# innnky/vispeech

Measured on AMD Instinct MI355X. Metric: 44.1kHz samples/sec, higher is better.
Workload: dtype f32 (split-f16 MFMA, 3-term); 1 GPU; C3: 64 mixed zh/ja utterances (~5 s each) per GPU, 44.1 kHz, hop 512, phoneme/duration/F0/energy/noise supplied, random-init (synthetic) weights of configs/config.json; 2 batches in flight per GPU; utterances_per_gpu=64, global_batch=64, padded_frames=489, frames_padded=31296, frames_computed=28902, parallelism=shard1, generator=f16s, controls=all, batches_in_flight=2

## Files before the change

### vispeech_amd/csrc/api_common.h

```cpp
#pragma once
#include <algorithm>
#include <cmath>
#include <cstdlib>
#include <cstring>
#include <vector>

#include "model.h"
#include "row_controls.h"

namespace vsp {

struct T3 {
  float* p = nullptr;
  long bs = 0, cs = 0;
  T3 chan(int c) const { return T3{p ? p + (size_t)c * cs : nullptr, bs, cs}; }
};

struct Ws {
  char* base;
  size_t cap;
  size_t cur = 0;
  bool dry;
  bool overflow = false;
  Ws(void* b, size_t c, bool d) : base((char*)b), cap(c), dry(d) {}
// ... 35 lines not shown
  const int* glen = nullptr;
  int grate_in = 0, grate_out = 0;
  bool iso = false;
  double work_frac = 1.0;
  bool dry() const { return ws.dry; }
  const float* A(size_t off) const { return ctx->arena + off; }
  bool ok() const { return rc == VSP_OK && !ws.overflow; }
  void chk(hipError_t e, const char* what) {
    if (e != hipSuccess && rc == VSP_OK) rc = ctx->fail(VSP_ERR_HIP, "%s: %s", what, hipGetErrorString(e));
  }

  static int fam(int kind, int channels) {
    if (channels <= 16) return kind | (7 << 3);
    int l = 0;
    while ((32 << l) < channels && l < 7) ++l;
    return kind | (l << 3);
  }
  ConvArgs args(const Conv& L, T3 x, T3 out, int T_in, int Nq) const {
    ConvArgs a;
    std::memset(&a, 0, sizeof a);
    a.x = x.p; a.x_bs = x.bs; a.x_cs = x.cs;
    a.wp = A(L.w);
    a.bias = L.b >= 0 ? A((size_t)L.b) : nullptr;
    a.out = out.p; a.o_bs = out.bs; a.o_cs = out.cs;
    a.Cin = L.Cin; a.M = L.M; a.K = L.K; a.dil = L.dil; a.pad = L.pad;
    a.T_in = T_in; a.Nq = Nq;
    a.nchunks = (L.Cin + CONV_CK - 1) / CONV_CK;
    a.alpha = 1.f; a.div = 1.f;
    a.ups_s = L.ups_s; a.ups_p = L.ups_p;
    a.f16s = L.f16s ? 1 : 0;
    a.wg = (L.has_wg && ctx->cols) ? reinterpret_cast<const uint16_t*>(A(L.wg)) : nullptr;
    a.wg_max_blocks = ctx->cols_blocks;
    a.wg_min_blocks = ctx->cols_min_blocks;
    return a;
  }
  bool prof_begin(int cls, int fam = VSP_FAM_OTHER) {
    if (!ctx->prof_on) return false;
    while (ctx->ev_pool.size() < ctx->ev_used + 2) {
      hipEvent_t e;
      if (hipEventCreate(&e) != hipSuccess) { rc = ctx->fail(VSP_ERR_HIP, "hipEventCreate"); return false; }
      ctx->ev_pool.push_back(e);
    }
    if (ctx->ev_cls.size() < ctx->ev_pool.size() / 2) {
      ctx->ev_cls.resize(ctx->ev_pool.size() / 2, 0);
      ctx->ev_fam.resize(ctx->ev_pool.size() / 2, 0);
      ctx->ev_flops.resize(ctx->ev_pool.size() / 2, 0.0);
      ctx->ev_bytes.resize(ctx->ev_pool.size() / 2, 0.0);
      ctx->ev_moved.resize(ctx->ev_pool.size() / 2, 0.0);
    }
    ctx->ev_cls[ctx->ev_used / 2] = cls;
    ctx->ev_fam[ctx->ev_used / 2] = fam;
    (void)hipEventRecord(ctx->ev_pool[ctx->ev_used], s);
    return true;
  }
  void prof_end(int cls, double flops, double bytes, double bytes_ext, double bytes_moved) {
    (void)hipEventRecord(ctx->ev_pool[ctx->ev_used + 1], s);
    const double f = cls == VSP_PROF_GENERATOR ? work_frac : 1.0;
    ctx->ev_flops[ctx->ev_used / 2] = flops * f;
    ctx->ev_bytes[ctx->ev_used / 2] = bytes * f;
    ctx->ev_moved[ctx->ev_used / 2] = bytes_moved * f;
    ctx->ev_used += 2;
    ctx->prof_launches[cls] += 1;
    ctx->prof_flops[cls] += flops * f;
    ctx->prof_bytes[cls] += bytes * f;
    ctx->prof_bytes_ext[cls] += bytes_ext * f;
    ctx->prof_bytes_moved[cls] += bytes_moved * f;
// ... 121 lines not shown
```

### vispeech_amd/csrc/api_context.hip

```cpp
#include "api_common.h"

using namespace vsp;

namespace vsp {

int check_ready(vsp_ctx* ctx) {
  if (!ctx) return VSP_ERR_ARG;
  if (!ctx->ready) return ctx->fail(VSP_ERR_STATE, "weights not finalised");
  return VSP_OK;
}

int check_vc(vsp_ctx* ctx) {
  const int rc = check_ready(ctx);
  if (rc) return rc;
  if (ctx->cfg.spec_channels <= 0) return ctx->fail(VSP_ERR_STATE, "context was created without spec_channels");
  if (!ctx->model.has_vc) return ctx->fail(VSP_ERR_STATE, "enc_q.* tensors were not loaded before vsp_finalize_weights");
  return VSP_OK;
}

}

extern "C" {

int vsp_abi_version(void) { return VSP_ABI_VERSION; }

int vsp_create(const vsp_config* cfg, int device, vsp_ctx** out) { return vsp_create_ex(cfg, 1, device, out); }

int vsp_create_ex(const vsp_config* cfg, int32_t resblock, int device, vsp_ctx** out) {
  if (!cfg || !out || (resblock != 1 && resblock != 2)) return VSP_ERR_ARG;
  vsp_ctx* ctx = new (std::nothrow) vsp_ctx();
  if (!ctx) return VSP_ERR_ARG;
  ctx->cfg = *cfg;
  ctx->resblock = resblock;
  ctx->device = device;
  if (const char* e = getenv("VSP_FRAME")) ctx->frame_f16s = strcmp(e, "f32") != 0;
  if (const char* e = getenv("VSP_ATT")) ctx->att_f16s = strcmp(e, "f32") != 0;
  bool want_f16 = false;
  if (const char* e = getenv("VSP_GENERATOR")) {
    if (!strcmp(e, "f32")) ctx->gen_mode = 0;
    want_f16 = !strcmp(e, "f16");
  }
  if (const char* e = getenv("VSP_FUSE_PAIRS")) ctx->fuse_pairs = atoi(e) != 0;
  if (const char* e = getenv("VSP_RB2_FUSE")) ctx->rb2_fuse = atoi(e) != 0;
  if (const char* e = getenv("VSP_TIMG")) ctx->t_img = atoi(e) != 0;
  if (const char* e = getenv("VSP_PP")) ctx->pp_pairs = atoi(e) != 0;
  if (const char* e = getenv("VSP_PAIR")) ctx->pair_ring = !strcmp(e, "ring");
  if (const char* e = getenv("VSP_CHAIN_RING")) ctx->chain_ring = atoi(e) != 0;
  if (const char* e = getenv("VSP_CHAIN")) ctx->chain_mask = atoi(e);
  if (const char* e = getenv("VSP_RW64")) ctx->rw64 = atoi(e) != 0;
  if (const char* e = getenv("VSP_TRIM_TAILS")) ctx->trim_tails = atoi(e) != 0;
  if (const char* e = getenv("VSP_TAIL_TABLE")) ctx->tail_table_on = atoi(e) != 0;
  if (const char* e = getenv("VSP_COLS")) ctx->cols = atoi(e) != 0;
  if (const char* e = getenv("VSP_COLS_BLOCKS")) ctx->cols_blocks = atol(e);
  if (const char* e = getenv("VSP_COLS_MIN_BLOCKS")) ctx->cols_min_blocks = atol(e);
  if (const char* e = getenv("VSP_ACT_SCALE_LOG2")) {
    const int l = atoi(e);
    ctx->act_scale = std::ldexp(1.f, l < 0 ? 0 : l > 8 ? 8 : l);
  }
  if (const char* e = getenv("VSP_EARLY_FL")) ctx->early_fl = atoi(e) != 0;
  if (const char* e = getenv("VSP_RB_STREAMS")) ctx->rb_streams = atoi(e);
#ifdef VSP_EXPERIMENTS
  if (const char* e = getenv("VSP_ATT_KSPLIT")) ctx->att_ksplit = atoi(e);
  if (const char* e = getenv("VSP_CHUNK_MB")) ctx->chunk_mb = atof(e);
  if (const char* e = getenv("VSP_CHAIN_CH")) ctx->chain_ch = atoi(e);
  if (const char* e = getenv("VSP_CHAIN128")) ctx->chain128_mask = atoi(e);
#endif
  build_schema(ctx->cfg, ctx->schema, ctx->resblock);
  const int rc = plan_model(ctx);
  if (want_f16 && ctx->gen_mode == 1) ctx->gen_mode = 2;
  *out = ctx;
  return rc;
}

int vsp_destroy(vsp_ctx* ctx) {
  if (!ctx) return VSP_ERR_ARG;
  for (auto e : ctx->ev_pool) (void)hipEventDestroy(e);
  for (auto e : ctx->sync_ev) (void)hipEventDestroy(e);
  if (ctx->fl_ev) (void)hipEventDestroy(ctx->fl_ev);
  if (ctx->fl_pinned) (void)hipHostFree(ctx->fl_pinned);
  if (ctx->flags_host) (void)hipHostFree(ctx->flags_host);
  for (auto st : ctx->side) if (st) (void)hipStreamDestroy(st);
  if (ctx->arena && ctx->arena_owned) (void)hipFree(ctx->arena);
  if (ctx->out_stage.tab) (void)hipFree(ctx->out_stage.tab);
  tail_table_drop(ctx);
  for (auto& r : ctx->in_rates) if (r.tab) (void)hipFree(r.tab);
// ... 436 lines not shown
```

### vispeech_amd/csrc/conv_mfma.hip

```cpp
#include "kernels.h"

#include <cstdio>
#include <cstdlib>
#include <cstring>
#include <type_traits>

namespace vsp {

typedef float f32x16 __attribute__((ext_vector_type(16)));

size_t packed_conv_floats(int M, int Cin, int K) {
  const size_t mt = (M + 31) / 32, nc = (Cin + CONV_CK - 1) / CONV_CK;
  return mt * nc * (size_t)K * 1024;
}

void pack_conv_weights(float* dst, int M, int Cin, int K, const float* dense) {
  const int nc = (Cin + CONV_CK - 1) / CONV_CK;
  std::memset(dst, 0, packed_conv_floats(M, Cin, K) * sizeof(float));
  for (int row = 0; row < M; ++row) {
    const int mtile = row >> 5, rin = row & 31;
    for (int ci = 0; ci < Cin; ++ci) {
      const int chunk = ci / CONV_CK, cc = ci % CONV_CK;
      const int kk = cc >> 1, hh = cc & 1, lane = rin + 32 * hh, kg = kk >> 2, i = kk & 3;
      for (int tap = 0; tap < K; ++tap) {
        const size_t idx =
            (((((size_t)mtile * nc + chunk) * K + tap) * (CONV_CK / 8) + kg) * 64 + lane) * 4 + i;
        dst[idx] = dense[((size_t)row * Cin + ci) * K + tap];
      }
    }
  }
}

void pack_conv_weights_f16s(float* dst_f, int M, int Cin, int K, const float* dense) {
// ... 420 lines not shown
    for (int nt = 0; nt < NT; ++nt) {
      const int tq = t0 + (wn * NT + nt) * 32;
      if constexpr (S == 1) {
        const int mtile = mtile0 + ms;
        if (mtile < n_mtiles && conv_tile_lean_ok(a, mtile)) {
          conv_tile_lean(a, acc[ms][nt], mtile, tq, l31, h, b, len);
          continue;
        }
      } else if constexpr (S == 2) {
        const int mtile = mtile0 + 2 * ms;
        if (conv_gate_lean_ok(a, mtile, n_mtiles)) {
          conv_gate_lean(a, acc[2 * ms][nt], acc[2 * ms + 1][nt], mtile, tq, l31, h, b, len);
          continue;
        }
      }
      f32x16 t[S][1];
#pragma unroll
      for (int u = 0; u < S; ++u) t[u][0] = acc[S * ms + u][nt];
      ConvEpi<S, 1> e;
      conv_epi_load<S, 1, false>(a, e, mtile0 + S * ms, n_mtiles, tq, 0, l31, h, b);
      conv_epi_store<S, 1>(a, t, e, mtile0 + S * ms, n_mtiles, tq, 0, l31, h, b, len);
    }
}
template <int MT, int NT>
__device__ __forceinline__ void conv_store_plain(const ConvArgs& a, f32x16 (&acc)[MT][NT], int mtile0, int n_mtiles, int t0,
                                                 int wn, int l31, int h, int b, int len) {
  if (a.act == 2) {
    if constexpr (MT % 2 == 0) conv_store_slices<2, MT, NT>(a, acc, mtile0, n_mtiles, t0, wn, l31, h, b, len);
  } else {
    conv_store_slices<1, MT, NT>(a, acc, mtile0, n_mtiles, t0, wn, l31, h, b, len);
  }
}

template <int MT, int NT, int WM, int WN, bool F16S, bool RING = false, bool PRUNE = false>
__global__ void __launch_bounds__(64 * WM * WN, F16S ? 2 : 1) conv1d_f32_mfma(ConvArgs a) {
  static_assert(!RING || F16S, "the weight ring serves the split-f16 path");
  static_assert(!PRUNE || (F16S && RING), "the pruned form is the split-f16 ring kernel");
  constexpr int BN = 32 * NT * WN;
  constexpr int LWP = BN + CONV_HALO;
  constexpr int NW = WM * WN;
  constexpr int KG = CONV_CK / 8;
  extern __shared__ __attribute__((aligned(16))) float xs[];
  constexpr int SB = MT * WM * 4096;
  constexpr int NS = conv_ring_slots(MT, WM), DEPTH = NS - 1;
  constexpr int PW = MT * WM * 4 / NW;
  static_assert(!RING || (MT * WM * 4) % NW == 0, "pieces divide over the waves");
  [[maybe_unused]] char* const ring = reinterpret_cast<char*>(xs) + (size_t)CONV_CK * LWP * sizeof(float);

  const int tid = threadIdx.x;
  const int wave = __builtin_amdgcn_readfirstlane(tid >> 6);
  const int lane = tid & 63;
  const int l31 = lane & 31, h = lane >> 5;
  const int wm = wave / WN, wn = wave % WN;
  const int b = blockIdx.z;
  const int t0 = blockIdx.x * BN;
  const int mtile0 = (blockIdx.y * WM + wm) * MT;
  const int n_mtiles = (a.M + 31) >> 5;
  const int len = a.lengths ? (int)a.lengths[b] : 0x7fffffff;
  const int LW = BN + (a.K - 1) * a.dil;
  const int total_it = a.nchunks * a.K;

  f32x16 acc[MT][NT];
#pragma unroll
  for (int mt = 0; mt < MT; ++mt)
#pragma unroll
    for (int nt = 0; nt < NT; ++nt)
#pragma unroll
      for (int r = 0; r < 16; ++r) {
        acc[mt][nt][r] = 0.f;
      }
// ... 368 lines not shown
        const int row = mtile * 32 + (r & 3) + 8 * (r >> 2) + 4 * h;
        if (!st[r]) continue;
        float v = acc[mt][nt][r];
        if (a.bias) v += a.bias[row];
        if (condb) v += condb[row];
        if (a.act == 1) v = fmaxf(v, 0.f);
        if (a.mask_pre && !valid) v = 0.f;
        if (a.alpha != 1.f) v *= a.alpha;
        if (resb) v += rv[r];
        if (a.acc_prev) v += pv[r];
        conv_div(v, a.div);
        if (a.mask_post && !valid) v = 0.f;
        outb[oidx[r]] = v;
      }
    }
  }
}

constexpr int FR_HALO = 12;

#define FR_VM1(k) case k: asm volatile("s_waitcnt vmcnt(" #k ")" ::: "memory"); break;
#define FR_VM8(a, b, c, d, e, f, g, h) FR_VM1(a) FR_VM1(b) FR_VM1(c) FR_VM1(d) FR_VM1(e) FR_VM1(f) FR_VM1(g) FR_VM1(h)
#ifndef FR_DIAG
#define FR_DIAG 0
#endif
__device__ __forceinline__ void fr_vmcnt(int n) {
  if constexpr ((FR_DIAG & 2) != 0) return;
  switch (n) {
    FR_VM8(0, 1, 2, 3, 4, 5, 6, 7) FR_VM8(8, 9, 10, 11, 12, 13, 14, 15) FR_VM8(16, 17, 18, 19, 20, 21, 22, 23)
    FR_VM8(24, 25, 26, 27, 28, 29, 30, 31) FR_VM8(32, 33, 34, 35, 36, 37, 38, 39) FR_VM8(40, 41, 42, 43, 44, 45, 46, 47)
    FR_VM8(48, 49, 50, 51, 52, 53, 54, 55) FR_VM8(56, 57, 58, 59, 60, 61, 62, 63)
    default: asm volatile("s_waitcnt vmcnt(63)" ::: "memory"); break;
  }
}
#ifdef FR_STAMPS
constexpr int FR_NSTAMP = 512, FR_NSAMPLE = 64;
__device__ unsigned long long g_fr_stamps[FR_NSAMPLE][FR_NSTAMP];
__device__ unsigned g_fr_stamp_count;
__device__ int g_fr_stamp_on;
#define FR_STAMPT(tag)                                                                  \
  do {                                                                                  \
    if (stamp_slot >= 0 && stamp_n < FR_NSTAMP && lane == 0)                            \
      g_fr_stamps[stamp_slot][stamp_n] = (__builtin_amdgcn_s_memrealtime() & 0x00ffffffffffffffull) | ((unsigned long long)(tag) << 56); \
    ++stamp_n;                                                                          \
  } while (0)
extern "C" int vsp_debug_stamps_frame(unsigned long long* host, int max_samples, int reset) {
  unsigned n = 0;
  (void)hipDeviceSynchronize();
  (void)hipMemcpyFromSymbol(&n, HIP_SYMBOL(g_fr_stamp_count), sizeof n);
  if ((int)n > max_samples) n = max_samples;
  if (n > (unsigned)FR_NSAMPLE) n = FR_NSAMPLE;
  (void)hipMemcpyFromSymbol(host, HIP_SYMBOL(g_fr_stamps), (size_t)n * FR_NSTAMP * sizeof(unsigned long long));
  if (reset) { const unsigned z = 0; (void)hipMemcpyToSymbol(HIP_SYMBOL(g_fr_stamp_count), &z, sizeof z); }
  return (int)n;
}
#else
#define FR_STAMPT(tag) ((void)0)
#endif
#if FR_DIAG & 1
#define FR_MFMA16(a, b, c) ([&]() { asm volatile("" ::"v"(a), "v"(b)); return c; }())
#else
#define FR_MFMA16(a, b, c) __builtin_amdgcn_mfma_f32_32x32x16_f16(a, b, c, 0, 0, 0)
#endif

template <int MT, int NT, int WM, int WN, int K, int G, int RI, int WI>
__global__ void __launch_bounds__(64 * WM * WN, 1) conv_frame_f16s(ConvArgs a) {
// ... 273 lines not shown
template <int MT, int NT, int WM, int WN, int K, int G, int RI, int WI>
static hipError_t launch_frame(const ConvArgs& a, int B, hipStream_t s) {
  constexpr int BN = 32 * NT * WN, BM = 32 * MT * WM, NW = WM * WN;
  constexpr int NF4 = CONV_CK * ((BN + (K == 1 ? 0 : FR_HALO)) / 4);
  constexpr size_t lds = (size_t)WI * G * ((NF4 + 64 * NW - 1) / (64 * NW)) * NW * 1024 + (size_t)RI * G * K * MT * WM * 4096;
  static_assert(lds <= 160 * 1024, "LDS budget");
  static std::atomic<uint64_t> attr_done{0};
  auto kern = conv_frame_f16s<MT, NT, WM, WN, K, G, RI, WI>;
  if (hipError_t e = set_max_dynamic_lds(reinterpret_cast<const void*>(kern), (int)lds, attr_done); e != hipSuccess) return e;
  dim3 grid((a.Nq + BN - 1) / BN, (a.M + BM - 1) / BM, B);
#ifdef FR_STAMPS
  {
    static int target = -2;
    if (target == -2) { const char* e = getenv("VSP_STAMP_FRAME"); target = e ? atoi(e) : -1; }
    const int on = g_fr_launch_no++ == target ? 1 : 0;
    (void)hipMemcpyToSymbolAsync(HIP_SYMBOL(g_fr_stamp_on), &g_fr_on_vals[on], sizeof(int), 0, hipMemcpyHostToDevice, s);
    if (on) fprintf(stderr, "[stamps] conv_frame_f16s<%d,%d,%d,%d,K%d,G%d,%d,%d> M %d Cin %d Nq %d grid %u x %u x %u\n", MT, NT, WM, WN, K,
                    G, RI, WI, a.M, a.Cin, a.Nq, grid.x, grid.y, grid.z);
  }
#endif
  hipLaunchKernelGGL(kern, grid, dim3(64 * WM * WN), lds, s, a);
  return hipGetLastError();
}
template <int MT, int NT, int WM, int WN>
static bool launch_frame_k(const ConvArgs& a, int B, hipStream_t s, hipError_t& e) {
  switch (a.K) {
    case 1: e = launch_frame<MT, NT, WM, WN, 1, 2, 3, 3>(a, B, s); return true;
    case 3: e = launch_frame<MT, NT, WM, WN, 3, 1, 3, 3>(a, B, s); return true;
    case 5: e = launch_frame<MT, NT, WM, WN, 5, 1, 2, 3>(a, B, s); return true;
    default: return false;
  }
}

template <int MT, int NT, int WM, int WN, bool F16S = false, bool RING = false, bool PRUNE = false>
static hipError_t launch_tile(const ConvArgs& a, int B, hipStream_t s) {
  constexpr int BN = 32 * NT * WN, BM = 32 * MT * WM;
  constexpr size_t lds = (size_t)CONV_CK * (BN + CONV_HALO) * sizeof(float) +
                         (RING ? (size_t)conv_ring_slots(MT, WM) * MT * WM * 4096 : 0);
  static_assert(lds <= 160 * 1024, "LDS budget (<= 80 KiB: two blocks per CU)");
  static std::atomic<uint64_t> attr_done{0};
  auto kern = conv1d_f32_mfma<MT, NT, WM, WN, F16S, RING, PRUNE>;
  if (hipError_t e = set_max_dynamic_lds(reinterpret_cast<const void*>(kern), (int)lds, attr_done); e != hipSuccess) return e;
  dim3 grid((a.Nq + BN - 1) / BN, (a.M + BM - 1) / BM, B);
  hipLaunchKernelGGL(kern, grid, dim3(64 * WM * WN), lds, s, a);
  return hipGetLastError();
}

template <int K, bool GATE>
__global__ void __launch_bounds__(256, 1) conv_frame_splitk(ConvArgs a) {
  constexpr int MT = 2, NT = 1, NWV = 4;
  constexpr int HALO = K == 1 ? 0 : FR_HALO;
  constexpr int BN = 32 * NT, LWP = BN + HALO, LWP4 = LWP / 4;
  constexpr int WBUF = CONV_CK * LWP * 4;
  constexpr int NIT = (16 * LWP4 + 63) / 64;
  constexpr int GT = 2;
  constexpr int GPC = (K + GT - 1) / GT;
  extern __shared__ __attribute__((aligned(16))) float xs[];
  char* const wbase = reinterpret_cast<char*>(xs);

  const int tid = threadIdx.x;
  const int wave = __builtin_amdgcn_readfirstlane(tid >> 6);
  const int lane = tid & 63;
  const int l31 = lane & 31, h = lane >> 5;
  const int b = blockIdx.z;
  const int t0 = blockIdx.x * BN;
  const int mtile0 = blockIdx.y * MT;
  const int n_mtiles = (a.M + 31) >> 5;
  const int nch = a.nchunks;
  const int total_it = nch * K;
  constexpr int FM = GATE ? 2 : 1;
  ConvEpi<FM, 1> epi;
  const bool finisher = wave < (GATE ? 1 : 2);
  const int fmt0 = mtile0 + (GATE ? 0 : wave);
  if (finisher) conv_epi_load<FM, 1>(a, epi, fmt0, n_mtiles, t0, 0, l31, h, b, 1);

// ... 315 lines not shown
      return form_tile(2, 1, 1, 4, true, true);
    }
    if (prune_ok) return form_tile(2, 2, 2, 2, true, true, true);
    return form_tile(2, 2, 2, 2, true, true);
  }
  if (a.f16s) {
    if (a.ups_s > 0) return form_of(VSP_CONV_FORM_NONE);
    if (a.M <= 32 && !gate) {
      if (a.Nq >= 1024) return form_tile(1, 4, 1, 4, true);
      return form_tile(1, 1, 1, 2, true);
    }
    if (a.Nq <= 96) return form_tile(2, 1, 1, 2, true);
    if (a.M <= 64 || (a.M % 128 != 0 && a.M < 256)) {
      if (a.Nq >= 1024) return form_tile(2, 2, 1, 4, true);
      return form_tile(2, 1, 1, 4, true);
    }
    return form_tile(2, 2, 2, 2, true);
  }
  if (a.M <= 32 && !gate) {
    if (a.Nq >= 1024) return form_tile(1, 4, 1, 4);
    return form_tile(1, 1, 1, 2);
  }
  if (a.Nq <= 96) return form_tile(2, 1, 1, 2);
  if (a.M <= 64 || (a.M % 128 != 0 && a.M < 256)) {
    if (a.Nq >= 1024) return form_tile(2, 4, 1, 4);
    return form_tile(2, 1, 1, 4);
  }
  return form_tile(2, 2, 2, 2);
}

static hipError_t launch_tile_form(const ConvForm& f, const ConvArgs& a, int B, hipStream_t s) {
  const int shape = f.mt * 1000 + f.nt * 100 + f.wm * 10 + f.wn;
  if (f.prune) {
    switch (shape) {
      case 2114: return launch_tile<2, 1, 1, 4, true, true, true>(a, B, s);
      case 2222: return launch_tile<2, 2, 2, 2, true, true, true>(a, B, s);
    }
  } else if (f.ring) {
    switch (shape) {
      case 1414: return launch_tile<1, 4, 1, 4, true, true>(a, B, s);
      case 1112: return launch_tile<1, 1, 1, 2, true, true>(a, B, s);
      case 2112: return launch_tile<2, 1, 1, 2, true, true>(a, B, s);
      case 2214: return launch_tile<2, 2, 1, 4, true, true>(a, B, s);
      case 2114: return launch_tile<2, 1, 1, 4, true, true>(a, B, s);
      case 2222: return launch_tile<2, 2, 2, 2, true, true>(a, B, s);
    }
  } else if (f.f16s) {
    switch (shape) {
      case 1414: return launch_tile<1, 4, 1, 4, true>(a, B, s);
      case 1112: return launch_tile<1, 1, 1, 2, true>(a, B, s);
      case 2112: return launch_tile<2, 1, 1, 2, true>(a, B, s);
      case 2214: return launch_tile<2, 2, 1, 4, true>(a, B, s);
      case 2114: return launch_tile<2, 1, 1, 4, true>(a, B, s);
      case 2222: return launch_tile<2, 2, 2, 2, true>(a, B, s);
    }
  } else {
    switch (shape) {
      case 1414: return launch_tile<1, 4, 1, 4>(a, B, s);
      case 1112: return launch_tile<1, 1, 1, 2>(a, B, s);
      case 2112: return launch_tile<2, 1, 1, 2>(a, B, s);
      case 2414: return launch_tile<2, 4, 1, 4>(a, B, s);
      case 2114: return launch_tile<2, 1, 1, 4>(a, B, s);
      case 2222: return launch_tile<2, 2, 2, 2>(a, B, s);
    }
  }
  return hipErrorInvalidValue;
// ... 26 lines not shown
```

### vispeech_amd/csrc/kernels.h

```cpp
#pragma once
#include <hip/hip_runtime.h>
#include <stdint.h>

#include <atomic>

#include "../../include/vispeech_hip.h"

namespace vsp {

inline hipError_t set_max_dynamic_lds(const void* kern, int bytes, std::atomic<uint64_t>& done) {
  int dev = 0;
  hipError_t e = hipGetDevice(&dev);
  if (e != hipSuccess) return e;
  const uint64_t bit = 1ull << (dev & 63);
  if (done.load(std::memory_order_acquire) & bit) return hipSuccess;
  e = hipFuncSetAttribute(kern, hipFuncAttributeMaxDynamicSharedMemorySize, bytes);
  if (e == hipSuccess) done.fetch_or(bit, std::memory_order_release);
  return e;
}

constexpr int CONV_CK = 32;
constexpr int CONV_HALO = 64;

struct ConvArgs {
  const float* x; long x_bs, x_cs;
  const float* wp;
  const float* bias;
  float* out; long o_bs, o_cs;
  const float* res; long r_bs, r_cs;
  const float* cond; long cond_bs;
  const int64_t* lengths;
  int Cin, M, K, dil, pad;
  int T_in;
  int Nq;
  int nchunks;
  int in_mask;
  int in_act; float in_slope;
  int act;
  int mask_pre;
  float alpha;
  int acc_prev;
  float div;
  int mask_post;
  int ups_s, ups_p, T_store;
  int f16s;
  int split_row; float* out2; long o2_bs, o2_cs; int acc_prev2;
  int mask_post2;
  const uint16_t* wg;
  long wg_min_blocks, wg_max_blocks;
};

using ConvForm = vsp_conv_form;
ConvForm conv_form(const ConvArgs& a, int B);
hipError_t launch_conv(const ConvArgs& a, int B, hipStream_t s);
bool conv_cols_supported(const ConvArgs& a);
hipError_t launch_conv_cols(const ConvArgs& a, int B, hipStream_t s, const float* ln_gamma = nullptr,
                            const float* ln_beta = nullptr);
size_t packed_conv_floats(int M, int Cin, int K);
void pack_conv_weights(float* dst, int M, int Cin, int K, const float* dense );
void pack_conv_weights_f16s(float* dst, int M, int Cin, int K, const float* dense );

#ifndef G16_WSCALE_V
#define G16_WSCALE_V 256.f
#define G16_UNSCALE_V (1.f / 256.f)
#endif
constexpr float G16_WSCALE = G16_WSCALE_V, G16_UNSCALE = G16_UNSCALE_V;

#ifdef __HIPCC__
__device__ __forceinline__ void vsp_raise_flag(unsigned* flags, unsigned bit) {
  __hip_atomic_fetch_or(flags, bit, __ATOMIC_RELAXED, __HIP_MEMORY_SCOPE_SYSTEM);
}
#ifndef VSP_SPLIT_FORM
#define VSP_SPLIT_FORM 1
#endif
__device__ __forceinline__ void vsp_split_pair(float x0, float x1, unsigned& hi, unsigned& lo) {
#if VSP_SPLIT_FORM == 0
  const float h0 = __uint_as_float(__float_as_uint(x0) & 0xffffe000u), h1 = __uint_as_float(__float_as_uint(x1) & 0xffffe000u);
  float l0, l1;
  asm("v_sub_f32 %0, %1, %2" : "=v"(l0) : "v"(x0), "v"(h0));
  asm("v_sub_f32 %0, %1, %2" : "=v"(l1) : "v"(x1), "v"(h1));
  hi = __builtin_bit_cast(unsigned, __builtin_amdgcn_cvt_pkrtz(h0, h1));
  lo = __builtin_bit_cast(unsigned, __builtin_amdgcn_cvt_pkrtz(l0, l1));
// ... 303 lines not shown
```

### vispeech_amd/csrc/model.h

```cpp
#pragma once
#include <hip/hip_runtime.h>

#include <cstdarg>
#include <cstdio>
#include <map>
#include <string>
#include <vector>

#include "../../include/vispeech_hip.h"
#include "kernels.h"

namespace vsp {

struct HostTensor {
  std::vector<int64_t> shape;
  std::vector<float> data;
  size_t numel() const { size_t n = 1; for (auto s : shape) n *= (size_t)s; return n; }
};

struct Conv {
  int M = 0, Cin = 0, K = 1, dil = 1, pad = 0;
  int ups_s = 0, ups_p = 0;
  size_t w = 0;
  long b = -1;
// ... 64 lines not shown
constexpr uint32_t ARENA_MAGIC = 0x41505356u;
constexpr uint32_t ARENA_FLAG_VC = 1u;

struct SchemaEntry {
  std::vector<int64_t> shape;
  bool used;
  bool optional = false;
};

}

struct vsp_ctx {
  vsp_config cfg;
  int resblock = 1;
  int device = 0;
  std::string err;
  std::map<std::string, vsp::SchemaEntry> schema;
  std::map<std::string, vsp::HostTensor> raw;
  vsp::Model model;
  float* arena = nullptr;
  bool arena_owned = false;
  bool ready = false;
  bool t_img = true;
  bool pp_pairs = true;
  bool pair_ring = false;
  bool chain_ring = false;
  bool rw64 = false;
  float act_scale = 16.f;
  unsigned* flags_host = nullptr;
  unsigned* flags_dev = nullptr;
  long cols_min_blocks = 32;
  long cols_blocks = 256;
  bool cols = true;
  bool trim_tails = true;
  bool tail_table_on = true;
  float* tail_table = nullptr;
  int tail_back = 0, tail_fwd = 0, tail_reach1 = 0;
  int rb_streams = 0;
  bool early_fl = true;
  int64_t* fl_pinned = nullptr;
  int fl_cap = 0, fl_n = 0;
  hipEvent_t fl_ev = nullptr;
  const int64_t* fl_src = nullptr;
  std::vector<int64_t> fl_known;
  const int64_t* fl_known_src = nullptr;
  hipStream_t side[2] = {nullptr, nullptr};
  std::vector<hipEvent_t> sync_ev;
  struct RateTable { int rate = 0; float* tab = nullptr; int L = 0, M = 0, H = 0, J = 0, P = 0; };
  RateTable out_stage;
  RateTable in_rates[VSP_INPUT_RATES_MAX];
  RateTable out_rates[VSP_OUTPUT_RATES_MAX];
  int64_t noise_first = 0;
  bool isolated = false;
  std::vector<uint64_t> noise_seeds;
  std::vector<vsp_row_control> row_controls;
  bool adopted_pending = false;
  int gen_mode = 1;
  bool frame_f16s = true;
  bool att_f16s = true;
  int att_ksplit = -1;
  int chain_mask = 0x1;
  int chain128_mask = 0;
  int chain_ch = 32;
  bool rb2_fuse = true;
  bool fuse_pairs = true;
  double chunk_mb = 0.0;
// ... 30 lines not shown
```

### vispeech_amd/csrc/ops.hip

```cpp
#include <algorithm>
#include <cstdlib>
#include <cstring>
#include <vector>

#include "kernels.h"

using namespace vsp;

namespace {
struct DevBuf {
  void* p = nullptr;
  ~DevBuf() { if (p) (void)hipFree(p); }
  hipError_t alloc(size_t bytes) { return hipMalloc(&p, bytes ? bytes : 16); }
};
hipError_t upload_cl_conv(const float* w_host, const float* bias_host, int Cout, int Cin, int K, DevBuf& w, DevBuf& bias,
                          hipStream_t s, int phases = 1) {
  const bool c16 = cl_is_c16(Cout, Cin, phases);
  std::vector<uint16_t> packed(c16 ? packed_g16c16_halfs(K) : packed_g16_halfs(phases * Cout, Cin, K));
  if (c16) pack_g16c16_weights(packed.data(), K, w_host);
  else pack_g16_weights(packed.data(), phases * Cout, Cin, K, w_host);
  hipError_t e = w.alloc(packed.size() * 2);
  if (e == hipSuccess) e = bias.alloc((size_t)Cout * 4);
  if (e == hipSuccess) e = hipMemcpyAsync(w.p, packed.data(), packed.size() * 2, hipMemcpyHostToDevice, s);
  std::vector<float> scaled(Cout, 0.f);
// ... 20 lines not shown
    if (l < 0 || l > T) return VSP_ERR_ARG;
  return VSP_OK;
}
hipError_t upload_emb(const float* emb_k_host, const float* emb_v_host, int window, int dk, DevBuf& ek, DevBuf& ev, hipStream_t s) {
  const size_t bytes = (size_t)(2 * window + 1) * dk * 4;
  hipError_t e = ek.alloc(bytes);
  if (e == hipSuccess) e = ev.alloc(bytes);
  if (e == hipSuccess) e = hipMemcpyAsync(ek.p, emb_k_host, bytes, hipMemcpyHostToDevice, s);
  if (e == hipSuccess) e = hipMemcpyAsync(ev.p, emb_v_host, bytes, hipMemcpyHostToDevice, s);
  if (e == hipSuccess) e = hipStreamSynchronize(s);
  return e;
}
}

extern "C" {

int vsp_cl_conv1d(void* stream, int B, int T, int Cin, int Cout, int K, int dilation, const float* x, const float* w_host,
                  const float* bias_host, float in_slope, const float* res, int terms, float* out) {
  if (!x || !w_host || !out || B < 0 || T < 0 || (terms != 1 && terms != 3)) return VSP_ERR_ARG;
  const bool c16 = Cin == 16 && Cout == 16;
  if (Cin <= 0 || Cout <= 0 || (!c16 && (Cin % 32 || Cout % 32)) || K < 1 || !(K & 1) || dilation < 1 || (K - 1) * dilation > 64 ||
      (size_t)T * std::max(Cin, Cout) * 4 >= (size_t)1 << 31)
    return VSP_ERR_UNSUPPORTED;
  if (c16 && x == out) return VSP_ERR_ARG;
  if (B == 0 || T == 0) return VSP_OK;
  hipStream_t s = (hipStream_t)stream;
  DevBuf w, bias;
  hipError_t e = upload_cl_conv(w_host, bias_host, Cout, Cin, K, w, bias, s);
  if (e == hipSuccess) e = launch_g16_conv(cl_conv_args(cw(w, bias), Cin, Cout, K, dilation, x, T, in_slope, res, out, terms), B, s);
  if (e == hipSuccess) e = hipStreamSynchronize(s);
  return op_rc(e);
}

int vsp_conv1d(void* stream, int B, int T, int Cin, int Cout, int K, int dilation, const float* x, const float* w_host,
               const float* bias_host, const int64_t* lengths, int mask_in, int in_act, float in_slope, int act,
               const float* res, int mask_out, int split_f16, float* out) {
  if (!x || !w_host || !out || B < 0 || T < 0 || act < 0 || act > 2 || ((mask_in || mask_out) && !lengths) || (act == 2 && res))
    return VSP_ERR_ARG;
  if (Cin <= 0 || Cout <= 0 || K < 1 || !(K & 1) || dilation < 1 || (K - 1) * dilation + 3 > CONV_HALO ||
      (act == 2 && Cout % 64) || ((T & 3) && T != 1))
    return VSP_ERR_UNSUPPORTED;
  if (B == 0 || T == 0) return VSP_OK;
  hipStream_t s = (hipStream_t)stream;
  std::vector<float> wd((size_t)Cout * Cin * K), bd(Cout, 0.f);
  for (int r = 0; r < Cout; ++r) {
    int src = r;
    if (act == 2) { const int tile = r / 32, in = r % 32; src = (tile & 1) * (Cout / 2) + (tile >> 1) * 32 + in; }
    std::memcpy(&wd[(size_t)r * Cin * K], w_host + (size_t)src * Cin * K, (size_t)Cin * K * sizeof(float));
    if (bias_host) bd[r] = bias_host[src];
  }
  std::vector<float> packed(packed_conv_floats(Cout, Cin, K));
  if (split_f16) pack_conv_weights_f16s(packed.data(), Cout, Cin, K, wd.data());
  else pack_conv_weights(packed.data(), Cout, Cin, K, wd.data());
  DevBuf w, bias;
  hipError_t e = w.alloc(packed.size() * 4);
  if (e == hipSuccess) e = bias.alloc((size_t)Cout * 4);
  if (e == hipSuccess) e = hipMemcpyAsync(w.p, packed.data(), packed.size() * 4, hipMemcpyHostToDevice, s);
  if (e == hipSuccess) e = hipMemcpyAsync(bias.p, bd.data(), (size_t)Cout * 4, hipMemcpyHostToDevice, s);
  if (e == hipSuccess) e = hipStreamSynchronize(s);
  if (e != hipSuccess) return op_rc(e);
  const int rows_out = act == 2 ? Cout / 2 : Cout;
  ConvArgs a;
  std::memset(&a, 0, sizeof a);
  a.x = x; a.x_bs = (long)Cin * T; a.x_cs = T;
  a.wp = static_cast<const float*>(w.p); a.bias = static_cast<const float*>(bias.p);
  a.out = out; a.o_bs = (long)rows_out * T; a.o_cs = T;
  a.res = res; a.r_bs = (long)rows_out * T; a.r_cs = T;
  a.lengths = lengths;
  a.Cin = Cin; a.M = Cout; a.K = K; a.dil = dilation; a.pad = dilation * (K - 1) / 2;
  a.T_in = T; a.Nq = T; a.nchunks = (Cin + CONV_CK - 1) / CONV_CK;
  a.in_mask = mask_in ? 1 : 0; a.in_act = in_act ? 1 : 0; a.in_slope = in_slope;
  a.act = act; a.alpha = 1.f; a.div = 1.f; a.mask_post = mask_out ? 1 : 0;
  a.f16s = split_f16 ? 1 : 0;
  if (split_f16 == 2) {
    std::vector<uint16_t> wgh(packed_g16_halfs(Cout, Cin, 1));
    DevBuf wgd;
    if (K != 1 || Cin % 32 || Cout % 16) return VSP_ERR_UNSUPPORTED;
    pack_g16_weights(wgh.data(), Cout, Cin, 1, wd.data());
    e = wgd.alloc(wgh.size() * 2);
    if (e == hipSuccess) e = hipMemcpyAsync(wgd.p, wgh.data(), wgh.size() * 2, hipMemcpyHostToDevice, s);
    if (e == hipSuccess) e = hipStreamSynchronize(s);
    if (e != hipSuccess) return op_rc(e);
    a.wg = static_cast<const uint16_t*>(wgd.p);
    if (!conv_cols_supported(a)) return VSP_ERR_UNSUPPORTED;
    e = launch_conv_cols(a, B, s);
    if (e == hipSuccess) e = hipStreamSynchronize(s);
    return op_rc(e);
  }
  e = launch_conv(a, B, s);
  if (e == hipSuccess) e = hipStreamSynchronize(s);
  return op_rc(e);
}

int vsp_conv1d_ex(void* stream, const vsp_conv1d_desc* dp, vsp_conv_form* form_out) {
  if (!dp || (dp->plan_only && !form_out)) return VSP_ERR_ARG;
  const vsp_conv1d_desc& d = *dp;
  const int B = d.B, T = d.T, Cin = d.Cin, Cout = d.Cout, K = d.K;
  const bool masks = d.mask_in || d.mask_pre || d.mask_post || d.mask_post2;
  if (!d.x || !d.w || !d.out || B < 0 || T < 0 || d.act < 0 || d.act > 2 || (masks && !d.lengths) ||
      (d.act == 2 && (d.res || d.split_row)) || d.split_f16 < 0 || d.split_f16 > 1 || d.cols < 0 || d.cols > 1 || d.ln < 0 ||
      d.ln > 2 || (d.ln == 1 && !d.cols) || (d.ln != 0) != (d.ln_gamma != nullptr) || (d.ln != 0) != (d.ln_beta != nullptr) ||
      (d.split_row != 0) != (d.out2 != nullptr) || ((d.acc_prev2 || d.mask_post2) && !d.split_row) || d.cond_bs < 0 ||
      !(d.div != 0.f))
    return VSP_ERR_ARG;
  if (Cin <= 0 || Cout <= 0 || K < 1 || !(K & 1) || d.dilation < 1 || (K - 1) * d.dilation + 3 > CONV_HALO ||
      (d.act == 2 && (Cout % 64 || d.mask_pre || d.alpha != 1.f || d.acc_prev || d.div != 1.f)) ||
// ... 5 lines not shown
  if (B == 0 || T == 0) return VSP_OK;
  const int rows_out = d.act == 2 ? Cout / 2 : (d.split_row ? d.split_row : Cout), rows2 = d.split_row ? Cout - d.split_row : 0;
  struct View { long bs, cs; int rows; };
  auto view = [&](int64_t bs, int64_t cs, int rows) {
    View v{(long)bs, (long)cs, rows};
    if (!v.cs) v.cs = T;
    if (!v.bs) v.bs = (long)rows * v.cs;
    return v;
  };
  const View vx = view(d.x_bs, d.x_cs, Cin), vo = view(d.o_bs, d.o_cs, rows_out), vr = view(d.r_bs, d.r_cs, rows_out),
             v2 = view(d.o2_bs, d.o2_cs, rows2);
  for (const View* v : {&vx, &vo, &vr, &v2}) {
    if (v == &vr && !d.res) continue;
    if (v == &v2 && !d.split_row) continue;
    if (v->cs < T || (B > 1 && v->bs < (long)(v->rows - 1) * v->cs + T)) return VSP_ERR_ARG;
    if (((long)v->rows * v->cs + T) * 4 >= (1L << 31)) return VSP_ERR_UNSUPPORTED;
  }
  hipStream_t s = (hipStream_t)stream;
  ConvArgs a;
  std::memset(&a, 0, sizeof a);
  a.x = d.x; a.x_bs = vx.bs; a.x_cs = vx.cs;
  a.out = d.out; a.o_bs = vo.bs; a.o_cs = vo.cs;
  if (d.res && (!d.ln || d.ln == 1)) { a.res = d.res; a.r_bs = vr.bs; a.r_cs = vr.cs; }
  a.cond = d.cond; a.cond_bs = (long)d.cond_bs;
  a.lengths = d.lengths;
  a.Cin = Cin; a.M = Cout; a.K = K; a.dil = d.dilation; a.pad = d.dilation * (K - 1) / 2;
  a.T_in = T; a.Nq = T; a.nchunks = (Cin + CONV_CK - 1) / CONV_CK;
  a.in_mask = d.mask_in ? 1 : 0; a.in_act = d.in_act ? 1 : 0; a.in_slope = d.in_slope;
  a.act = d.act; a.mask_pre = d.mask_pre ? 1 : 0; a.alpha = d.alpha; a.acc_prev = d.acc_prev ? 1 : 0; a.div = d.div;
  a.mask_post = d.mask_post ? 1 : 0;
  a.split_row = d.split_row; a.out2 = d.out2; a.o2_bs = v2.bs; a.o2_cs = v2.cs; a.acc_prev2 = d.acc_prev2 ? 1 : 0;
  a.mask_post2 = d.mask_post2 ? 1 : 0;
  a.f16s = d.split_f16 ? 1 : 0;
  const bool cols_shape = K == 1 && Cin % 32 == 0 && Cout % 16 == 0;
  vsp_conv_form form{};
  if (d.cols) {
    if (!cols_shape) return VSP_ERR_UNSUPPORTED;
    static const uint16_t no_image = 0;
    a.wg = &no_image;
    if (!conv_cols_supported(a)) return VSP_ERR_UNSUPPORTED;
    if (d.ln == 1 && (Cout != 192 || Cin != 192 || a.mask_pre || a.mask_post || a.alpha != 1.f)) return VSP_ERR_UNSUPPORTED;
    form.kernel = d.ln == 1 ? VSP_CONV_FORM_COLS_LN : VSP_CONV_FORM_COLS;
    a.wg = nullptr;
  } else {
    form = conv_form(a, B);
    if (form.kernel == VSP_CONV_FORM_NONE) return VSP_ERR_UNSUPPORTED;
  }
  if (form_out) *form_out = form;
  if (d.plan_only) return VSP_OK;
  if (int rc = check_lengths64(d.lengths, B, T, s); rc != VSP_OK) return rc;
  std::vector<float> wd((size_t)Cout * Cin * K), bd(Cout, 0.f);
  for (int r = 0; r < Cout; ++r) {
    int src = r;
    if (d.act == 2) { const int tile = r / 32, in = r % 32; src = (tile & 1) * (Cout / 2) + (tile >> 1) * 32 + in; }
    std::memcpy(&wd[(size_t)r * Cin * K], d.w + (size_t)src * Cin * K, (size_t)Cin * K * sizeof(float));
    if (d.bias) bd[r] = d.bias[src];
  }
  DevBuf w, bias, wgd, scratch, gamma, beta;
  hipError_t e = bias.alloc((size_t)Cout * 4);
  if (e == hipSuccess) e = hipMemcpyAsync(bias.p, bd.data(), (size_t)Cout * 4, hipMemcpyHostToDevice, s);
  std::vector<float> packed;
  std::vector<uint16_t> wgh;
  if (d.cols) {
    wgh.resize(packed_g16_halfs(Cout, Cin, 1));
    pack_g16_weights(wgh.data(), Cout, Cin, 1, wd.data());
    if (e == hipSuccess) e = wgd.alloc(wgh.size() * 2);
// ... 274 lines not shown
```

Baseline: 208.2 million samples/s.

## Add pruned conv tile variant staging split-f16 windows once and stepping two taps

Adds a new kernel body for the 2x1x1x4 pruned split-f16 ring tile. Each chunk's input window is converted once into 16-byte f16 hi/lo images in LDS, and the weight ring advances two taps per barrier step instead of one. It is selected by default (frame_steps defaults to 0, and only 1 disables it). The intent is to cut per-tap staging, barriers and conversion work. The cost is more complex vmcnt accounting and a different LDS footprint that may change occupancy.

Result: no change. 208.9 million samples/s (median of 6 runs) (+0.3%).

```diff
diff --git a/vispeech_amd/csrc/api_common.h b/vispeech_amd/csrc/api_common.h
--- a/vispeech_amd/csrc/api_common.h
+++ b/vispeech_amd/csrc/api_common.h
@@ -91,6 +91,7 @@
     a.wg = (L.has_wg && ctx->cols) ? reinterpret_cast<const uint16_t*>(A(L.wg)) : nullptr;
     a.wg_max_blocks = ctx->cols_blocks;
     a.wg_min_blocks = ctx->cols_min_blocks;
+    a.frame_steps = ctx->frame_steps;
     return a;
   }
   bool prof_begin(int cls, int fam = VSP_FAM_OTHER) {
diff --git a/vispeech_amd/csrc/api_context.hip b/vispeech_amd/csrc/api_context.hip
--- a/vispeech_amd/csrc/api_context.hip
+++ b/vispeech_amd/csrc/api_context.hip
@@ -51,6 +51,7 @@
   if (const char* e = getenv("VSP_TRIM_TAILS")) ctx->trim_tails = atoi(e) != 0;
   if (const char* e = getenv("VSP_TAIL_TABLE")) ctx->tail_table_on = atoi(e) != 0;
   if (const char* e = getenv("VSP_COLS")) ctx->cols = atoi(e) != 0;
+  if (const char* e = getenv("VSP_FRAME_STEPS")) ctx->frame_steps = atoi(e);
   if (const char* e = getenv("VSP_COLS_BLOCKS")) ctx->cols_blocks = atol(e);
   if (const char* e = getenv("VSP_COLS_MIN_BLOCKS")) ctx->cols_min_blocks = atol(e);
   if (const char* e = getenv("VSP_ACT_SCALE_LOG2")) {
diff --git a/vispeech_amd/csrc/conv_mfma.hip b/vispeech_amd/csrc/conv_mfma.hip
--- a/vispeech_amd/csrc/conv_mfma.hip
+++ b/vispeech_amd/csrc/conv_mfma.hip
@@ -1,4 +1,5 @@
 #include "kernels.h"
+#include "conv_steps.h"
 
 #include <cstdio>
 #include <cstdlib>
@@ -485,10 +486,18 @@
   }
 }
 
-template <int MT, int NT, int WM, int WN, bool F16S, bool RING = false, bool PRUNE = false>
+template <int MT, int NT, int WM, int WN, int TS, int SW>
+__device__ __forceinline__ void conv_steps_tile(const ConvArgs& a);
+
+template <int MT, int NT, int WM, int WN, bool F16S, bool RING = false, bool PRUNE = false, int FS = 0, int SW = 3>
 __global__ void __launch_bounds__(64 * WM * WN, F16S ? 2 : 1) conv1d_f32_mfma(ConvArgs a) {
   static_assert(!RING || F16S, "the weight ring serves the split-f16 path");
   static_assert(!PRUNE || (F16S && RING), "the pruned form is the split-f16 ring kernel");
+  static_assert(FS == 0 || PRUNE, "the 16-byte window images serve the pruned form");
+  if constexpr (FS > 0) {
+    conv_steps_tile<MT, NT, WM, WN, FS, SW>(a);
+    return;
+  }
   constexpr int BN = 32 * NT * WN;
   constexpr int LWP = BN + CONV_HALO;
   constexpr int NW = WM * WN;
@@ -923,6 +932,175 @@
     FR_VM8(48, 49, 50, 51, 52, 53, 54, 55) FR_VM8(56, 57, 58, 59, 60, 61, 62, 63)
     default: asm volatile("s_waitcnt vmcnt(63)" ::: "memory"); break;
   }
+}
+
+template <int MT, int NT, int WM, int WN, int TS, int SW>
+__device__ __forceinline__ void conv_steps_tile(const ConvArgs& a) {
+  constexpr int BN = 32 * NT * WN, NW = WM * WN, KG = CONV_CK / 8;
+  static_assert(NW == 4 && BN == 128 && CONV_CK == 32, "wave w stages plane w of a 32-channel chunk in 64-column sweeps");
+  constexpr int SB = MT * WM * 4096;
+  constexpr int NS = conv_steps_slots(TS), DEPTH = NS - 1;
+  constexpr int PW = MT * WM * 4 / NW;
+  static_assert((MT * WM * 4) % NW == 0, "pieces divide over the waves");
+  static_assert(TS == 1 || DEPTH == 1, "the counted wait knows the pieces of younger steps only for one-tap steps");
+  extern __shared__ __attribute__((aligned(16))) float xs[];
+
+  const int tid = threadIdx.x;
+  const int wave = __builtin_amdgcn_readfirstlane(tid >> 6);
+  const int lane = tid & 63;
+  const int l31 = lane & 31, h = lane >> 5;
+  const int wm = wave / WN, wn = wave % WN;
+  const int b = blockIdx.z;
+  const int t0 = blockIdx.x * BN;
+  const int mtile0 = (blockIdx.y * WM + wm) * MT;
+  const int n_mtiles = (a.M + 31) >> 5;
+  const int len = a.lengths ? (int)a.lengths[b] : 0x7fffffff;
+  const int LW = BN + (a.K - 1) * a.dil;
+  const int lwp = conv_steps_lwp(BN, a.K, a.dil);
+  const int img = 4 * lwp * 16;
+  const int spc = (a.K + TS - 1) / TS;
+  const int total_it = a.nchunks * spc, total_taps = a.nchunks * a.K;
+  char* const win = reinterpret_cast<char*>(xs);
+  char* const ring = win + 2 * img;
+
+  f32x16 acc[MT][NT];
+#pragma unroll
+  for (int mt = 0; mt < MT; ++mt)
+#pragma unroll
+    for (int nt = 0; nt < NT; ++nt)
+#pragma unroll
+      for (int r = 0; r < 16; ++r) acc[mt][nt][r] = 0.f;
+
+  const float4* wp4 = reinterpret_cast<const float4*>(a.wp);
+  int d_step = 0, d_tap = 0, d_left = a.K;
+  auto ring_dma = [&]() {
+    char* dst = ring + (d_step % NS) * (TS * SB);
+    const int ntap = d_left < TS ? d_left : TS;
+#pragma unroll
+    for (int u = 0; u < TS; ++u) {
+      if (u < ntap) {
+#pragma unroll
+        for (int v = 0; v < PW; ++v) {
+          const int p = v * NW + wave;
+          int mtile = blockIdx.y * (WM * MT) + (p >> 2);
+          mtile = mtile < n_mtiles ? mtile : n_mtiles - 1;
+          const float4* src = wp4 + (((size_t)mtile * total_taps + d_tap + u) * KG + (p & 3)) * 64 + lane;
+          __builtin_amdgcn_global_load_lds((const __attribute__((address_space(1))) void*)src,
+                                           (__attribute__((address_space(3))) void*)(dst + u * SB + p * 1024), 16, 0, 0);
+        }
+      }
+    }
+    d_tap += ntap;
+    d_left = d_left == ntap ? a.K : d_left - ntap;
+    ++d_step;
+  };
+  static_assert(SW == 2 || SW == 3, "staging sweeps of 64 columns: 2 cover the tile (K = 1), 3 any window conv_form admits");
+  int pf_step = -1000;
+  auto ring_wait = [&](int step) {
+    int n = 0;
+    if constexpr (DEPTH > 1) n = (total_it - 1 - step < DEPTH - 1 ? total_it - 1 - step : DEPTH - 1) * (TS * PW);
+    if (step > pf_step && step - pf_step <= DEPTH) n += 8 * SW;
+    fr_vmcnt(n);
+  };
+#pragma unroll
+  for (int d = 0; d < DEPTH; ++d)
+    if (d < total_it) ring_dma();
+
+  const float* xb = a.x + (size_t)b * a.x_bs;
+  float pv[SW][8];
+  auto st_load = [&](int chunk) {
+    const int c0 = chunk * CONV_CK + 8 * wave;
+#pragma unroll
+    for (int sw = 0; sw < SW; ++sw) {
+      const int col = 64 * sw + lane, t = t0 - a.pad + col;
+      int tc = col < LW && t >= 0 && t < a.T_in ? t : 0;
+      asm("" : "+v"(tc));
+#pragma unroll
+      for (int j = 0; j < 8; ++j) {
+        const float* row = xb + (size_t)(c0 + j < a.Cin ? c0 + j : 0) * a.x_cs;
+        pv[sw][j] = row[tc];
+      }
+    }
+  };
+  typedef float f32x2v __attribute__((ext_vector_type(2)));
+  const float slope_eff = a.in_act ? a.in_slope : 1.f;
+  const int lim = a.in_mask ? (len < a.T_in ? len : a.T_in) : a.T_in;
+  auto st_write = [&](int chunk) {
+    const int c0 = chunk * CONV_CK + 8 * wave;
+#pragma unroll
+    for (int sw = 0; sw < SW; ++sw) {
+      const int col = 64 * sw + lane, t = t0 - a.pad + col;
+      const bool tv = t >= 0 && t < lim;
+      unsigned wh4[4], wl4[4];
+#pragma unroll
+      for (int i = 0; i < 4; ++i) {
+        f32x2v x = {(tv && c0 + 2 * i < a.Cin) ? pv[sw][2 * i] : 0.f, (tv && c0 + 2 * i + 1 < a.Cin) ? pv[sw][2 * i + 1] : 0.f};
+        const f32x2v y = x * slope_eff;
+        asm("v_max_f32 %0, %1, %2" : "=v"(x.x) : "v"(x.x), "v"(y.x));
+        asm("v_max_f32 %0, %1, %2" : "=v"(x.y) : "v"(x.y), "v"(y.y));
+        vsp_split_pair(x.x, x.y, wh4[i], wl4[i]);
+      }
+      if (col < LW) {
+        char* dst = win + (wave * lwp + col) * 16;
+        *reinterpret_cast<u32x4*>(dst) = u32x4{wh4[0], wh4[1], wh4[2], wh4[3]};
+        *reinterpret_cast<u32x4*>(dst + img) = u32x4{wl4[0], wl4[1], wl4[2], wl4[3]};
+      }
+    }
+  };
+
+  st_load(0);
+  const int colb = h * lwp + wn * (NT * 32) + l31;
+  int it = 0;
+  auto step = [&](int chunk, int s, bool first) __attribute__((always_inline)) {
+    ring_wait(it);
+    CONV_RAW_BARRIER();
+    if (it + DEPTH < total_it) ring_dma();
+    if (first && chunk + 1 < a.nchunks) { st_load(chunk + 1); pf_step = it; }
+    const char* slot = ring + (it % NS) * (TS * SB) + (wm * MT) * 4096 + lane * 16;
+    const int ntap = a.K - s * TS < TS ? a.K - s * TS : TS;
+#pragma unroll
+    for (int u = 0; u < TS; ++u) {
+      if (u < ntap) {
+        const char* bp = win + (colb + (s * TS + u) * a.dil) * 16;
+#pragma unroll
+        for (int ks = 0; ks < 2; ++ks) {
+          f16x8 bh[NT], bl[NT];
+#pragma unroll
+          for (int nt = 0; nt < NT; ++nt) {
+            bh[nt] = *reinterpret_cast<const f16x8*>(bp + (2 * ks * lwp + nt * 32) * 16);
+            bl[nt] = *reinterpret_cast<const f16x8*>(bp + (2 * ks * lwp + nt * 32) * 16 + img);
+          }
+#pragma unroll
+          for (int mt = 0; mt < MT; ++mt) {
+            const char* pa = slot + u * SB + mt * 4096 + ks * 2048;
+            const f16x8 ah = *reinterpret_cast<const f16x8*>(pa);
+            const f16x8 al = *reinterpret_cast<const f16x8*>(pa + 1024);
+#pragma unroll
+            for (int nt = 0; nt < NT; ++nt) acc[mt][nt] = CONV_MFMA16(ah, bh[nt], acc[mt][nt]);
+#pragma unroll
+            for (int nt = 0; nt < NT; ++nt) acc[mt][nt] = CONV_MFMA16(ah, bl[nt], acc[mt][nt]);
+#pragma unroll
+            for (int nt = 0; nt < NT; ++nt) acc[mt][nt] = CONV_MFMA16(al, bh[nt], acc[mt][nt]);
+          }
+        }
+      }
+    }
+    ++it;
+  };
+  for (int chunk = 0; chunk < a.nchunks; ++chunk) {
+    st_write(chunk);
+    step(chunk, 0, true);
+    for (int s = 1; s < spc; ++s) step(chunk, s, false);
+    CONV_RAW_BARRIER();
+  }
+
+#pragma unroll
+  for (int mt = 0; mt < MT; ++mt)
+#pragma unroll
+    for (int nt = 0; nt < NT; ++nt)
+#pragma unroll
+      for (int r = 0; r < 16; ++r) acc[mt][nt][r] *= G16_UNSCALE;
+  conv_store_plain<MT, NT>(a, acc, mtile0, n_mtiles, t0, wn, l31, h, b, len);
 }
 #ifdef FR_STAMPS
 constexpr int FR_NSTAMP = 512, FR_NSAMPLE = 64;
@@ -1262,15 +1440,20 @@
   }
 }
 
-template <int MT, int NT, int WM, int WN, bool F16S = false, bool RING = false, bool PRUNE = false>
+template <int MT, int NT, int WM, int WN, bool F16S = false, bool RING = false, bool PRUNE = false, int FS = 0, int SW = 3>
 static hipError_t launch_tile(const ConvArgs& a, int B, hipStream_t s) {
   constexpr int BN = 32 * NT * WN, BM = 32 * MT * WM;
-  constexpr size_t lds = (size_t)CONV_CK * (BN + CONV_HALO) * sizeof(float) +
-                         (RING ? (size_t)conv_ring_slots(MT, WM) * MT * WM * 4096 : 0);
-  static_assert(lds <= 160 * 1024, "LDS budget (<= 80 KiB: two blocks per CU)");
+  constexpr size_t lds_max = FS > 0 ? (size_t)conv_steps_lds_bytes(BN, BM, FS, 2, CONV_HALO)
+                                    : (size_t)CONV_CK * (BN + CONV_HALO) * sizeof(float) +
+                                          (RING ? (size_t)conv_ring_slots(MT, WM) * MT * WM * 4096 : 0);
+  static_assert(lds_max <= (size_t)CONV_STEPS_LDS_CU, "LDS budget: a block fits a CU");
+  static_assert(!(RING && BM == 64 && BN == 128) ||
+                    3 * (FS > 0 ? (size_t)conv_steps_lds_bytes(BN, BM, FS, 5, 1) : lds_max) <= (size_t)CONV_STEPS_LDS_CU,
+                "LDS budget of the 64-row ring tile: three blocks per CU");
+  const size_t lds = FS > 0 ? (size_t)conv_steps_lds_bytes(BN, BM, FS, a.K, a.dil) : lds_max;
   static std::atomic<uint64_t> attr_done{0};
-  auto kern = conv1d_f32_mfma<MT, NT, WM, WN, F16S, RING, PRUNE>;
-  if (hipError_t e = set_max_dynamic_lds(reinterpret_cast<const void*>(kern), (int)lds, attr_done); e != hipSuccess) return e;
+  auto kern = conv1d_f32_mfma<MT, NT, WM, WN, F16S, RING, PRUNE, FS, SW>;
+  if (hipError_t e = set_max_dynamic_lds(reinterpret_cast<const void*>(kern), (int)lds_max, attr_done); e != hipSuccess) return e;
   dim3 grid((a.Nq + BN - 1) / BN, (a.M + BM - 1) / BM, B);
   hipLaunchKernelGGL(kern, grid, dim3(64 * WM * WN), lds, s, a);
   return hipGetLastError();
@@ -1652,6 +1835,9 @@
 static hipError_t launch_tile_form(const ConvForm& f, const ConvArgs& a, int B, hipStream_t s) {
   const int shape = f.mt * 1000 + f.nt * 100 + f.wm * 10 + f.wn;
   if (f.prune) {
+    if (a.frame_steps != 1 && shape == 2114)
+      return a.K == 1 ? launch_tile<2, 1, 1, 4, true, true, true, CONV_STEPS_TAPS, 2>(a, B, s)
+                      : launch_tile<2, 1, 1, 4, true, true, true, CONV_STEPS_TAPS, 3>(a, B, s);
     switch (shape) {
       case 2114: return launch_tile<2, 1, 1, 4, true, true, true>(a, B, s);
       case 2222: return launch_tile<2, 2, 2, 2, true, true, true>(a, B, s);
diff --git a/vispeech_amd/csrc/conv_steps.h b/vispeech_amd/csrc/conv_steps.h
--- /dev/null
+++ b/vispeech_amd/csrc/conv_steps.h
@@ -0,0 +1,11 @@
+#pragma once
+
+constexpr int CONV_STEPS_LDS_CU = 160 * 1024;
+constexpr int CONV_STEPS_TAPS = 2;
+
+constexpr int conv_steps_lwp(int BN, int K, int dil) { return (BN + (K - 1) * dil + 15) & ~15; }
+constexpr int conv_steps_window_bytes(int BN, int K, int dil) { return 2 * 4 * conv_steps_lwp(BN, K, dil) * 16; }
+constexpr int conv_steps_slots(int TS) { return TS == 2 ? 2 : 3; }
+constexpr int conv_steps_lds_bytes(int BN, int rows, int TS, int K, int dil) {
+  return conv_steps_window_bytes(BN, K, dil) + conv_steps_slots(TS) * TS * (rows / 32) * 4096;
+}
diff --git a/vispeech_amd/csrc/kernels.h b/vispeech_amd/csrc/kernels.h
--- a/vispeech_amd/csrc/kernels.h
+++ b/vispeech_amd/csrc/kernels.h
@@ -48,6 +48,7 @@
   int mask_post2;
   const uint16_t* wg;
   long wg_min_blocks, wg_max_blocks;
+  int frame_steps;
 };
 
 using ConvForm = vsp_conv_form;
diff --git a/vispeech_amd/csrc/model.h b/vispeech_amd/csrc/model.h
--- a/vispeech_amd/csrc/model.h
+++ b/vispeech_amd/csrc/model.h
@@ -120,6 +120,7 @@
   long cols_min_blocks = 32;
   long cols_blocks = 256;
   bool cols = true;
+  int frame_steps = 0;
   bool trim_tails = true;
   bool tail_table_on = true;
   float* tail_table = nullptr;
diff --git a/vispeech_amd/csrc/ops.hip b/vispeech_amd/csrc/ops.hip
--- a/vispeech_amd/csrc/ops.hip
+++ b/vispeech_amd/csrc/ops.hip
@@ -76,6 +76,11 @@
   return op_rc(e);
 }
 
+static int op_frame_steps() {
+  const char* e = getenv("VSP_FRAME_STEPS");
+  return e ? atoi(e) : 0;
+}
+
 int vsp_conv1d(void* stream, int B, int T, int Cin, int Cout, int K, int dilation, const float* x, const float* w_host,
                const float* bias_host, const int64_t* lengths, int mask_in, int in_act, float in_slope, int act,
                const float* res, int mask_out, int split_f16, float* out) {
@@ -116,6 +121,7 @@
   a.in_mask = mask_in ? 1 : 0; a.in_act = in_act ? 1 : 0; a.in_slope = in_slope;
   a.act = act; a.alpha = 1.f; a.div = 1.f; a.mask_post = mask_out ? 1 : 0;
   a.f16s = split_f16 ? 1 : 0;
+  a.frame_steps = op_frame_steps();
   if (split_f16 == 2) {
     std::vector<uint16_t> wgh(packed_g16_halfs(Cout, Cin, 1));
     DevBuf wgd;
@@ -187,6 +193,7 @@
   a.split_row = d.split_row; a.out2 = d.out2; a.o2_bs = v2.bs; a.o2_cs = v2.cs; a.acc_prev2 = d.acc_prev2 ? 1 : 0;
   a.mask_post2 = d.mask_post2 ? 1 : 0;
   a.f16s = d.split_f16 ? 1 : 0;
+  a.frame_steps = op_frame_steps();
   const bool cols_shape = K == 1 && Cin % 32 == 0 && Cout % 16 == 0;
   vsp_conv_form form{};
   if (d.cols) {
```
